# marbl/parsnp

Hardware: AMD Instinct MI355X
Metric: genomes/sec (MUM+LCB end-to-end) (higher is better)
Workload: dtype int32

## Files before the change

parsnp_amd/csrc/engine/engine_core.h:

```cpp
#pragma once
#include <algorithm>
#include <atomic>
#include <chrono>
#include <cstdint>
#include <cstdio>
#include <cstdlib>
#include <cstring>
#include <memory>
#include <mutex>
#include <new>
#include <string>
#include <thread>
#include <vector>

#include "kernels.h"
#include "store_kernels.h"
#include "dense_kernels.h"
#include "index_kernels.h"
#include "snp_kernels.h"

namespace pm {

struct HostPool {
    void* (*alloc_fn)(size_t) = nullptr;
// ... 171 lines not shown
    static constexpr size_t kCtrErr = kCtrBase;
    static constexpr size_t kCtrGrouped = kCtrBase + 2;
    static constexpr size_t kCtrWide = kCtrBase + 3;
    static constexpr size_t kCtrWideWords = 3;
    static constexpr size_t kCtrOverflow = kCtrBase + 6;
    static constexpr size_t kCtrLost = kCtrBase + 7;
    static constexpr size_t kCtrWords = kCtrBase + 8;
    static_assert(kCtrErr < kCtrGrouped && kCtrGrouped < kCtrWide && kCtrWide + kCtrWideWords <= kCtrOverflow && kCtrOverflow < kCtrLost && kCtrLost < kCtrWords,
                  "the words of the counter block are distinct and inside it");

private:
    struct CallHint { int64_t units = 0, ncand = 0, nok = 0; };
    struct StoreCounts { int64_t ms_count, rg_count, layout_rows, rg_pkey_init; };
    StoreCounts store_mark() const { return StoreCounts{ms_count, rg_count, layout_rows, rg_pkey_init}; }
    void store_rewind(const StoreCounts& m) { ms_count = m.ms_count; rg_count = m.rg_count; layout_rows = m.layout_rows; rg_pkey_init = m.rg_pkey_init; }
    void store_reset() { store_rewind(StoreCounts{0, 0, -1, 0}); }

    struct SearchCall {
        const int64_t nreg; const int64_t* const starts; const int64_t* const lens; const int32_t* const minsize; BatchResult* const out;
        const bool want_events, mumi; const GapBatch* const gb;
        bool from_store = false;
        int nq = 0, no_small = 0, lbits = 0;
        size_t nrow = 0, regz = 0, bytes_R = 0, bytes_pre = 0;
        int64_t npairs = 0, npos = 0, tsize = 0, fwords = 0, tsize_clear = 0, fwords_clear = 0, nbk = 0, npos_bucketed = 0, nchunks = 0, centries = 0, nwv = 0;
        RegionInfo* R = nullptr; int64_t *posbase = nullptr, *cbase = nullptr, *stage = nullptr;
        std::vector<int64_t> bbase;
        uint32_t* d_err = nullptr;
        int64_t nflag = 0; uint64_t ovf_cap = 0; bool index_counts_read = false;
        CallHint none; CallHint* hint = nullptr;
        int64_t nunits = 0; bool units_known = false;
        size_t ev_guess = 0, slice_cap = 0, queue_cap = 0, grp_cap = 0;
        uint64_t nev = 0, nrest = 0, ngrp = 0, worst_slice = 0;
        uint32_t errbits = 0, sticky = 0;
        bool first_form = false, wide_form = false, grouping = false, by_buckets = false, sharded = false;
        uint64_t *skey = nullptr, *sval = nullptr;
        const int64_t* ncand_p = nullptr; bool anchor_guess = false;
        bool exact = false, anchor_call = false;
        int64_t ncand_i = 0, nok = 0; uint64_t ncand = 0; size_t nokz = 0; const int64_t* nok_p = nullptr;
        std::vector<uint64_t> counts, qcounts; int64_t nunits_live = 0;
        int32_t verdict = 0;
        std::vector<int32_t> reg_h; int64_t counts_h[2] = {0, 0};
    };
    static constexpr int kNext = 1, kRepeat = 2;

    int run_once(int64_t nreg, const int64_t* starts, const int64_t* lens, const int32_t* minsize, BatchResult* out, bool want_events,
                 bool mumi, const GapBatch* gb = nullptr) {
        SearchCall c{nreg, starts, lens, minsize, out, want_events, mumi, gb};
        int rc = plan_call(c);
        if (rc != kNext) return rc;
        upload_and_clear(c);
        if ((rc = build_index(c)) != kNext) return rc;
        if ((rc = count_units(c)) != kNext) return rc;
        if ((rc = search_events(c)) != kNext) return rc;
        order_events(c);
        if (mumi) return mumi_tail(c);
        if ((rc = master_ep(c)) != kNext) return rc;
        return candidate_tail(c);
    }

    int plan_call(SearchCall& c) {
        const int64_t nreg = c.nreg; const int64_t* const starts = c.starts; const int64_t* const lens = c.lens; const int32_t* const minsize = c.minsize;
        BatchResult* const out = c.out; const GapBatch* const gb = c.gb;
        timing.clear();
        const int nq = c.nq = ngen - 1;
        out->nregions = nreg; out->nq = nq; out->total = 0;
        out->off.assign((size_t)nreg + 1, 0);
        out->release();
// ... 123 lines not shown
    }

    void upload_and_clear(SearchCall& c) {
        const int64_t nreg = c.nreg, npos = c.npos, tsize = c.tsize, fwords = c.fwords, tsize_clear = c.tsize_clear, fwords_clear = c.fwords_clear, npairs = c.npairs, centries = c.centries;
        const int nq = c.nq;
        const size_t nrow = c.nrow, regz = c.regz, bytes_R = c.bytes_R, bytes_pre = c.bytes_pre;
        const GapBatch* const gb = c.gb; const bool from_store = c.from_store;
        RegionInfo* const R = c.R; int64_t* const posbase = c.posbase; int64_t* const cbase = c.cbase; int64_t* const stage = c.stage;
        be.mark("setup");
        ensure(d_R, regz);
        ensure(d_starts, nrow); ensure(d_lens, nrow);
        ensure(d_posbase, regz + 1); ensure(d_cbase, regz + 1);
        be.h2d_staged(d_R.p, R, bytes_R);
        be.h2d_staged(d_posbase.p, posbase, bytes_pre);
        be.h2d_staged(d_cbase.p, cbase, bytes_pre);
        if (!gb) {
            be.h2d_staged(d_starts.p, stage, sizeof(int64_t) * nrow);
            be.h2d_staged(d_lens.p, stage + nrow, sizeof(int64_t) * nrow);
        } else if (from_store) {
            ensure(d_list, regz);
            be.h2d_staged(d_list.p, stage, sizeof(int32_t) * regz);
            be.launch("gather_regions", (int64_t)nrow, GatherRegions{d_list.p, ngen, d_rg_start.p, d_rg_len.p, d_starts.p, d_lens.p});
        }
        ensure(d_counter, kCtrWords);
        uint32_t* d_err = c.d_err = (uint32_t*)(d_counter.p + kCtrErr);

        ensure(d_slots, (size_t)tsize); ensure(d_filter, (size_t)fwords);
        ensure(d_next, (size_t)std::max<int64_t>(npos, 1)); ensure(d_rep, (size_t)std::max<int64_t>(npos, 1));
        ensure(d_epm, (size_t)std::max<int64_t>(npos, 1) + 1);
        const int64_t nwv = c.nwv = (npos + 63) / 64;
        ensure(d_repeated, (size_t)(npos / 32 + 2));
        ensure(d_ucount, (size_t)npairs + 1); ensure(d_uoff, (size_t)npairs + 1);
        ensure(d_coarse, (size_t)std::max<int64_t>(centries, 1));
        ensure(d_wmask, (size_t)nwv + 1); ensure(d_wcount, (size_t)nwv + 1); ensure(d_woff, (size_t)nwv + 1);
        if (from_store) ensure(d_alg, 8 * (size_t)kAlgSets);
        ensure(d_dense, regz);
        {
            const ClearJob jobs[] = {
                {d_filter.p, sizeof(uint32_t) * (size_t)fwords_clear, 0}, {d_slots.p, sizeof(uint64_t) * (size_t)tsize_clear, 0xff}, {d_counter.p, 8 * kCtrWords, 0},
                {d_repeated.p, 4 * (size_t)(npos / 32 + 2), 0}, {d_coarse.p, 4 * (size_t)std::max<int64_t>(centries, 1), 0},
                {d_ucount.p + npairs, 8, 0}, {d_wcount.p + nwv, 8, 0}, {from_store ? d_alg.p : nullptr, from_store ? (size_t)64 * kAlgSets : 0, 0},
                {dense_mode ? nullptr : d_dense.p, dense_mode ? 0 : regz, 0}};
            be.clear_many(jobs, (int)(sizeof jobs / sizeof jobs[0]));
        }
        int64_t& nflag = c.nflag;
        if (dense_mode) {
            for (int64_t r = 0; r < nreg; r++) nflag += dense_h[(size_t)r] ? 1 : 0;
            be.h2d(d_dense.p, dense_h.data(), regz);
            last_dense_regions = nflag;
        }
        if (gb) be.launch("check_rows", (int64_t)nrow, CheckRows{d_R.p, d_starts.p, d_lens.p, ngen, d_glen, d_err});
        if (from_store) {
            be.launch_wave("alg_bytes", (nreg * nq + kAlgPairs - 1) / kAlgPairs, AlgBytes{d_R.p, d_lens.p, ngen, nreg * nq, d_alg.p});
        }
    }

    int build_index(SearchCall& c) {
        const int64_t nreg = c.nreg, npos = c.npos, nbk = c.nbk, npos_bucketed = c.npos_bucketed, nflag = c.nflag;
        const size_t regz = c.regz;
        const RegionInfo* const R = c.R; const std::vector<int64_t>& bbase = c.bbase; uint32_t* const d_err = c.d_err;
        be.mark("index");
        const uint64_t ovf_cap = c.ovf_cap = nbk > 0 ? (uint64_t)(index_overflow_cap > 0 ? index_overflow_cap : npos_bucketed / 32 + 1024) : 0;
        if (nbk > 0) {
            const int pbits = bits_for((uint64_t)npos), bbits = bits_for((uint64_t)nbk);
            if (pbits + bbits > 64) { error = "batch too large for 64-bit index keys"; return -5; }
            ensure(d_bkbase, regz + 1); ensure(d_ikey, (size_t)npos); ensure(d_ikey2, (size_t)npos); ensure(d_bkbegin, (size_t)nbk + 1); ensure(d_ovf, (size_t)ovf_cap);
            be.h2d(d_bkbase.p, bbase.data(), 8 * (regz + 1));
            be.launch("index_keys", npos, IndexKeys{P, d_R.p, nreg, d_posbase.p, d_bkbase.p, pbits, d_ikey.p, d_next.p, d_rep.p});
            if (!sort_keys_on(be, d_ikey.p, d_ikey2.p, (size_t)npos, pbits, pbits + bbits, 0)) {
                ensure(d_ikey3, (size_t)npos); ensure(d_ikey4, (size_t)npos);
                be.launch("index_key_buckets", npos, IndexKeyBuckets{d_ikey.p, pbits, d_ikey3.p});
                be.sort_pairs(d_ikey3.p, d_ikey4.p, d_ikey.p, d_ikey2.p, (size_t)npos, bbits);
            }
// ... 149 lines not shown
        uint32_t& errbits = c.errbits;
        errbits |= c.sticky;
        if (from_store) {
            alg_raw[0] = alg_raw[1] = alg_raw[2] = 0;
            for (int x = 0; x < kAlgSets; x++) for (int k = 0; k < 3; k++) alg_raw[k] += alg_sets[8 * x + k];
        }
        if (from_store) { last_alg[0] = (double)alg_raw[0] / 4.0; last_alg[1] = (double)alg_raw[1] / 2.0; last_alg[2] = (double)alg_raw[2] / 2.0; }
        if (errbits & kErrRows) { error = "region outside its genome"; return -2; }
        rest_cap_hint[nreg == 1] = queue_cap - 64;
        if (gb) hint.units = std::max<int64_t>(nunits_live, 1);
        last_rest = (int64_t)nrest;
        ev_cap_hint = (size_t)(nev + nev / 4);
        if (grouping) grp_cap_hint = (size_t)(ngrp + ngrp / 4);
        last_events = (int64_t)(nev + ngrp);
        last_grouped = (int64_t)ngrp;
        last_grouped_wide = wide_form ? (int64_t)counts[kCtrWide] : 0;
        last_handed_back = wide_form ? (int64_t)counts[kCtrWide + 1] : -1;
        last_wide_regions = wide_form ? (int64_t)counts[kCtrWide + 2] : 0;
        const bool sharded = c.sharded = coll.world > 1 || coll.device;
        if ((errbits & kErrWork) && !sharded) { budget_exceeded = true; error = "per-thread work budget exceeded (degenerate repeat structure in a region)"; return -5; }
        return kNext;
    }

    void order_events(SearchCall& c) {
        const int64_t nreg = c.nreg, npairs = c.npairs, npos = c.npos, nchunks = c.nchunks, centries = c.centries; const int nq = c.nq, lbits = c.lbits;
        const uint64_t ngrp = c.ngrp, worst_slice = c.worst_slice; const size_t slice_cap = c.slice_cap; const bool grouping = c.grouping;
        uint64_t& nev = c.nev;
        ensure(d_evkey2, std::max<size_t>(nev, 1)); ensure(d_evval2, std::max<size_t>(nev, 1));
        ensure_keep(d_evkey3, std::max<size_t>(ngrp + nev, 1), (size_t)ngrp); ensure_keep(d_evval3, std::max<size_t>(ngrp + nev, 1), (size_t)ngrp);
        const int keybits = bits_for((uint64_t)npairs) + lbits + 1;
        uint64_t *skey = c.skey = d_evkey3.p, *sval = c.sval = d_evval3.p;
        const int64_t nbuckets = (int64_t)nq * nchunks;
        const bool by_buckets = c.by_buckets = bucket_sort && nev > 0 && nbuckets < ((int64_t)1 << 31);
        ensure(d_lo, (size_t)npairs + 1);
        if (by_buckets) {
            ensure(d_bcount, (size_t)nbuckets + 1); ensure(d_bbegin, (size_t)nbuckets + 1); ensure(d_pbase, (size_t)npairs);
            int shift = 6;
            while (((uint64_t)1 << shift) < worst_slice) shift++;
            be.memset(d_bcount.p, 0, 8 * ((size_t)nbuckets + 1));
            be.launch("pair_bucket_base", npairs, PairBucketBase{nq, d_cbase.p, d_pbase.p});
            be.launch("event_bucket_count", (int64_t)kSlices << shift, EventBucketCount{d_evkey.p, d_counter.p, (uint64_t)slice_cap, shift, lbits, d_pbase.p, d_bcount.p});
            be.exclusive_scan(d_bcount.p, d_bbegin.p, (size_t)nbuckets + 1);
            be.launch("event_place", (int64_t)kSlices << shift,
                      EventPlace{d_evkey.p, d_evval.p, d_counter.p, (uint64_t)slice_cap, shift, lbits, d_pbase.p, d_bbegin.p, d_bcount.p, d_evkey3.p + ngrp, d_evval3.p + ngrp});
            be.launch("event_order", nbuckets, EventOrder{d_bbegin.p, nbuckets, d_evkey3.p + ngrp, d_evval3.p + ngrp});
        } else if (nev > 0) {
            be.launch("compact_events", (int64_t)nev, CompactEvents{d_evkey.p, d_evval.p, d_sliceoff.p, (uint64_t)slice_cap, d_evkey2.p, d_evval2.p});
            be.sort_pairs(d_evkey2.p, d_evkey3.p + ngrp, d_evval2.p, d_evval3.p + ngrp, (size_t)nev, keybits);
        }
        be.mark("scan");
        const int64_t nev_sorted = (int64_t)nev;
        nev += ngrp;
        if (by_buckets) be.launch("coarse_from_buckets", centries, CoarseFromBuckets{d_bbegin.p, d_cbase.p, nreg, nq, (int64_t)ngrp, d_coarse.p, d_lo.p, npairs, nev_sorted});
        else be.launch("pair_bounds", npairs, PairBounds{skey, (int64_t)nev, lbits, npairs, d_lo.p, (int64_t)ngrp});
        if (grouping) be.launch("grouped_bounds", npairs, GroupedBounds{d_gflag.p, d_glo.p, nq, d_lo.p});
        ensure_keep(d_state, std::max<size_t>(nev, 1), (size_t)ngrp); ensure_keep(d_emax, std::max<size_t>(nev, 1), (size_t)ngrp);
        const int64_t nsorted = (int64_t)(nev - ngrp);
        if (nsorted > 0) {
            const int64_t nwaves = (nsorted + kWaveEvents - 1) / kWaveEvents;
            ensure(d_wsummary, (size_t)nwaves);
            const WaveScanCore core{skey + ngrp, sval + ngrp, nsorted, lbits, d_R.p, nq, d_rep.p};
            be.launch_wave("wave_summary", nwaves, WaveSummary{core, d_wsummary.p});
            be.launch_wave("wave_scan", nwaves, WaveScan{core, d_wsummary.p, d_lo.p, (int64_t)ngrp, d_state.p + ngrp, d_emax.p + ngrp});
        }

        if (c.want_events) {
            ev_key_h.resize((size_t)nev); ev_val_h.resize((size_t)nev); rep_h.resize((size_t)npos);
            if (nev) { be.d2h(ev_key_h.data(), skey, 8 * (size_t)nev); be.d2h(ev_val_h.data(), sval, 8 * (size_t)nev); }
            if (npos) be.d2h(rep_h.data(), d_rep.p, 4 * (size_t)npos);
            ev_lbits = lbits;
        }
    }

    int widest_block() const {
        int widest = 0;
        for (int r = 0; r < coll.world; r++) { int a, b; shard_range(ngen, r, coll.world, &a, &b); widest = std::max(widest, b - a); }
        return std::max(widest, 1);
    }

    int mumi_tail(SearchCall& c) {
        const int64_t npairs = c.npairs; const int lbits = c.lbits; const bool sharded = c.sharded;
        uint64_t* const skey = c.skey; uint64_t* const sval = c.sval; uint32_t& errbits = c.errbits;
        be.mark("mumi_coverage");
        ensure(d_cov, (size_t)npairs);
        be.launch("mumi_coverage", npairs, MumiCoverage{d_R.p, skey, sval, d_lo.p, d_state.p, d_rep.p, lbits, ngen, d_cov.p});
        mumi_covered.resize((size_t)npairs);
        be.d2h(mumi_covered.data(), d_cov.p, 8 * (size_t)npairs);
        if (sharded) {
            const size_t per = (size_t)widest_block() + 1;
            std::vector<int64_t> send(per, 0), recv(per * (size_t)coll.world);
            for (int g = g_first; g < g_last; g++) send[(size_t)(g - g_first)] = mumi_covered[(size_t)(g - 1)];
            send[per - 1] = errbits;
            if (allgather_host(send.data(), (int64_t)(8 * send.size()), recv.data())) { error = "all-gather of MUMi coverage failed"; return -4; }
            for (int r = 0; r < coll.world; r++) {
                int a, b; shard_range(ngen, r, coll.world, &a, &b);
                for (int g = a; g < b; g++) mumi_covered[(size_t)(g - 1)] = recv[(size_t)r * per + (size_t)(g - a)];
// ... 1108 lines not shown
    template <class T> void ensure_keep(Buf<T>& b, size_t n, size_t keep) {
        if (n <= b.cap && b.p) return;
        if (std::find(all_bufs.begin(), all_bufs.end(), (BufBase*)&b) == all_bufs.end()) all_bufs.push_back(&b);
        const size_t want = n + n / 2 + 16;
        void* raw = be.alloc(want * sizeof(T));
        if (!raw) throw DeviceOutOfMemory{want * sizeof(T)};
        if (b.p && keep) { be.d2d(raw, b.p, keep * sizeof(T)); be.sync(); }
        if (b.raw) be.free(b.raw);
        b.raw = raw; b.p = (T*)raw; b.cap = want;
    }
    void collect_timing() { timing = be.collect(); }
    template <class T> static auto group_on(T& b, int) -> decltype(b.d2h_group(), void()) { b.d2h_group(); }
    template <class T> static void group_on(T&, long) {}
    template <class T> static auto flush_on(T& b, int) -> decltype(b.d2h_flush(), void()) { b.d2h_flush(); }
    template <class T> static void flush_on(T&, long) {}
    template <class T> static auto tune_copy_kernel(T& b, bool on, int) -> decltype(b.group_copies = on, true) { b.group_copies = on; return true; }
    template <class T> static bool tune_copy_kernel(T&, bool, long) { return true; }
    template <class T> static auto sort_keys_on(T& b, uint64_t* ki, uint64_t* ko, size_t n, int lo, int hi, int) -> decltype(b.sort_keys(ki, ko, n, lo, hi), true) { b.sort_keys(ki, ko, n, lo, hi); return true; }
    template <class T> static bool sort_keys_on(T&, uint64_t*, uint64_t*, size_t, int, int, long) { return false; }
    void group_downloads() { group_on(be, 0); }
    void flush_downloads() { flush_on(be, 0); }

    SeqBlock* blk = nullptr; int64_t* d_goff = nullptr; int64_t* d_glen = nullptr;
    Packed P{};
    size_t ev_cap_hint = 0, rest_cap_hint[2] = {0, 0}, grp_cap_hint = 0;
    std::vector<CallHint> call_hints;
    int64_t call_ordinal = 0;
    Buf<uint8_t> d_gflag; Buf<int64_t> d_glo;
    Buf<int64_t> d_bkbase, d_bkbegin, d_ovf; Buf<uint64_t> d_ikey, d_ikey2, d_ikey3, d_ikey4;
    Buf<RegionInfo> d_R; Buf<int64_t> d_starts, d_lens, d_posbase;
    Buf<uint64_t> d_slots; Buf<uint32_t> d_filter, d_repeated; Buf<int32_t> d_next, d_rep, d_run, d_epm;
    Buf<int64_t> d_ucount, d_uoff; Buf<UnitRec> d_units;
    Buf<uint64_t> d_counter, d_evkey, d_evval, d_evkey2, d_evval2, d_evkey3, d_evval3; Buf<int64_t> d_sliceoff;
    Buf<int64_t> d_lo, d_cov; Buf<EventAtK> d_state; Buf<PairState> d_wsummary; Buf<int32_t> d_emax;
    Buf<uint64_t> d_cand; Buf<GenomeAtK> d_at; Buf<uint8_t> d_ok; Buf<int32_t> d_ok_k, d_ok_lon, d_osp; Buf<uint8_t> d_ofwd;
    Buf<uint64_t> d_wmask; Buf<int64_t> d_wcount, d_woff;
    Buf<int64_t> d_bcount, d_bbegin, d_pbase;
    Buf<int64_t> d_okcnt, d_okpos, d_cbase; Buf<int32_t> d_coarse; Buf<int32_t> d_creg, d_ck, d_clon, d_csp; Buf<uint8_t> d_cfwd;
    Buf<uint32_t> d_cflags, d_dirty; Buf<int32_t> d_bmax, d_bmin;
    Buf<GenomeAtK> d_xsend, d_xrecv; Buf<uint8_t> d_hsend, d_hrecv;
    Buf<RestItem> d_rest; Buf<uint64_t> d_qcount;
    Buf<uint8_t> d_dense; Buf<int32_t> d_dfi, d_dlist, d_dlcp; Buf<int64_t> d_dstart, d_dhead, d_dfirst;
    Buf<uint64_t> d_dkey, d_dkey2, d_dval, d_dval2; Buf<uint32_t> d_drank[kDenseMaxLevels];
    Buf<int32_t> d_anchor_start, d_anchor_lon; Buf<uint32_t> d_anchor_flags;
    int64_t table_counter = 0;
    Buf<uint64_t> d_image;
    Buf<int64_t> d_un_blk, d_un_cnt, d_un_scan, d_un_tot; Buf<int32_t> d_un_out;
    Buf<uint64_t> d_snp_counts, d_snp_lo, d_snp_hi; Buf<uint8_t> d_snp_chunk; Buf<int64_t> d_snp_flag, d_snp_rank, d_snp_col; Buf<int32_t> d_snp_dist;
    Buf<uint8_t> d_ms_strand, d_ms_state, d_small8, d_o_strand; Buf<int32_t> d_ms_shift, d_ms_len, d_list, d_list2, d_j_min, d_j_max, d_o_start;
    Buf<int64_t> d_rg_start, d_rg_len, d_lay_off, d_lay_bits, d_v_row0, d_v_first, d_f_start, d_f_end, d_f_pack; Buf<RegInfo> d_rg_info; Buf<uint64_t> d_rg_count, d_once, d_twice;
    Buf<RowInfo> d_rowinfo; Buf<uint64_t> d_alg;
    Buf<int64_t> d_sd_cnt, d_sd_off; Buf<uint8_t> d_sd_keep;
    Buf<uint64_t> d_t_rem; Buf<uint8_t> d_t_done;
    Buf<int32_t> d_v_done, d_owner; Buf<uint8_t> d_v_defer, d_v_involved;
    Buf<uint64_t> d_t_left; uint64_t tangle_left[8] = {0, 0, 0, 0, 0, 0, 0, 0}; int tangle_ran = 0;
    Buf<int64_t> d_rg_pkey; Buf<OutsideWrite> d_outw; Buf<uint64_t> d_outw_count; int64_t rg_pkey_init = 0; uint64_t outside_writes_call = 0;
    Buf<ForeignRead> d_foreign; Buf<uint64_t> d_foreign_count, d_foreign_masks; Buf<int64_t> d_ms_key;
    size_t foreign_cap = 0; int64_t ms_key_rows = 0; uint64_t foreign_seen = 0;
    static constexpr size_t kHitCap = 256;
    Buf<uint64_t> d_hit_count, d_hit_owned, d_hit_present; Buf<int32_t> d_hits; Buf<uint8_t> d_recwords;
    Buf<int64_t> d_ch_flag, d_ch_pos, d_ch_head, d_ch_hpos, d_ch_survive, d_ch_spos, d_ch_hdr;
    Buf<uint64_t> d_ch_key, d_ch_val, d_ch_skey, d_ch_srow, d_ch_key2, d_ch_row2, d_ch_lcblen;
    Buf<uint8_t> d_ch_verdict, d_ch_outhead; Buf<int32_t> d_ch_outrow;
    Buf<int64_t> d_ch_back, d_ch_wflag, d_ch_wpos, d_ch_wlist, d_ch_wend; Buf<uint8_t> d_ch_wverdict, d_ch_wkeep;
    uint8_t* chain_host = nullptr; size_t chain_host_cap = 0; void* chain_event = nullptr; bool chain_pending = false; int64_t chain_cap = 0;
    size_t lay_words = 0, rg_cap_hint = 0;
    int64_t layout_rows = -1;
// ... 4 lines not shown
```

parsnp_amd/csrc/engine/kernels.h:

```cpp
#pragma once
#include <cstdint>

#if defined(__HIPCC__)
#define PM_HD __host__ __device__ inline
#else
#define PM_HD inline
#endif

namespace pm {

PM_HD int ctz64(uint64_t x) {
#if defined(__HIP_DEVICE_COMPILE__)
    return __ffsll((unsigned long long)x) - 1;
#else
    return __builtin_ctzll(x);
#endif
}
PM_HD int clz64(uint64_t x) {
#if defined(__HIP_DEVICE_COMPILE__)
    return __clzll((long long)x);
#else
    return __builtin_clzll(x);
#endif
}
// ... 1080 lines not shown

struct PairBucketBase {
    int32_t nq; const int64_t* cbase; int64_t* pbase;
    PM_HD void operator()(int64_t pair) const {
        const int64_t r = pair / nq; const int64_t g = pair % nq;
        pbase[pair] = (int64_t)nq * (cbase[r] - r) + g * (cbase[r + 1] - cbase[r] - 1);
    }
};
PM_HD int64_t bucket_of_key(uint64_t k, int lbits, const int64_t* pbase) {
    return pbase[k >> (lbits + 1)] + (int64_t)(((k >> 1) & ((1ull << lbits) - 1)) >> 8);
}
struct EventBucketCount {
    const uint64_t* key_in; const uint64_t* counters; uint64_t slice_cap; int shift; int lbits; const int64_t* pbase; int64_t* count;
    PM_HD void operator()(int64_t tid) const {
        const uint64_t sl = (uint64_t)tid >> shift, idx = (uint64_t)tid & ((1ull << shift) - 1);
        const bool active = idx < counters[sl * kSliceStride];
#if defined(__HIP_DEVICE_COMPILE__)
        const int lane = (int)__lane_id();
        const int64_t b = active ? bucket_of_key(key_in[sl * slice_cap + idx], lbits, pbase) : -1;
        const int64_t prev = ((int64_t)__shfl_up((int)(b >> 32), 1, 64) << 32) | (uint32_t)__shfl_up((int)(uint32_t)b, 1, 64);
        const bool head = active && (lane == 0 || prev != b);
        const unsigned long long heads = __ballot(head), act = __ballot(active);
        if (!head) return;
        const unsigned long long above = lane == 63 ? 0ull : heads & (~0ull << (lane + 1));
        const int upto = above ? __ffsll((long long)above) - 1 : __popcll(act);
        atomic_add64((uint64_t*)&count[b], (uint64_t)(upto - lane));
#else
        if (active) atomic_add64((uint64_t*)&count[bucket_of_key(key_in[sl * slice_cap + idx], lbits, pbase)], 1);
#endif
    }
};
struct EventPlace {
    const uint64_t* key_in; const uint64_t* val_in; const uint64_t* counters; uint64_t slice_cap; int shift; int lbits; const int64_t* pbase;
    const int64_t* begin; int64_t* count; uint64_t* key_out; uint64_t* val_out;
    PM_HD void operator()(int64_t tid) const {
        const uint64_t sl = (uint64_t)tid >> shift, idx = (uint64_t)tid & ((1ull << shift) - 1);
        const bool active = idx < counters[sl * kSliceStride];
        const uint64_t src = sl * slice_cap + idx;
#if defined(__HIP_DEVICE_COMPILE__)
        const int lane = (int)__lane_id();
        const uint64_t k = active ? key_in[src] : 0;
        const int64_t b = active ? bucket_of_key(k, lbits, pbase) : -1;
        const int64_t prev = ((int64_t)__shfl_up((int)(b >> 32), 1, 64) << 32) | (uint32_t)__shfl_up((int)(uint32_t)b, 1, 64);
        const bool head = active && (lane == 0 || prev != b);
        const unsigned long long heads = __ballot(head), act = __ballot(active);
        int64_t first = 0;
        if (head) {
            const unsigned long long above = lane == 63 ? 0ull : heads & (~0ull << (lane + 1));
            const int upto = above ? __ffsll((long long)above) - 1 : __popcll(act);
            const int64_t run = upto - lane;
            first = begin[b] + (int64_t)atomic_add64((uint64_t*)&count[b], (uint64_t)(-run)) - run;
        }
        const unsigned long long below = heads & (lane == 63 ? ~0ull : ((2ull << lane) - 1));
        const int mine = below ? 63 - __clzll((long long)below) : 0;
        first = ((int64_t)__shfl((int)(first >> 32), mine, 64) << 32) | (uint32_t)__shfl((int)(uint32_t)first, mine, 64);
        if (!active) return;
        const int64_t at = first + (lane - mine);
        key_out[at] = k; val_out[at] = val_in[src];
#else
        if (!active) return;
        const uint64_t k = key_in[src];
        const int64_t b = bucket_of_key(k, lbits, pbase);
        const int64_t at = begin[b] + (int64_t)atomic_add64((uint64_t*)&count[b], ~0ull) - 1;
        key_out[at] = k; val_out[at] = val_in[src];
#endif
    }
};
struct EventOrder {
    const int64_t* begin; int64_t nbuckets; uint64_t* key; uint64_t* val;
    PM_HD void operator()(int64_t b) const {
        const int64_t a = begin[b], n = begin[b + 1] - a;
        if (n < 2) return;
        uint64_t* k = key + a; uint64_t* v = val + a;
        if (n == 2) {
            const uint64_t k0 = k[0], k1 = k[1];
            if (k1 < k0) { const uint64_t v0 = v[0], v1 = v[1]; k[0] = k1; k[1] = k0; v[0] = v1; v[1] = v0; }
            return;
        }
        if (n <= 8) {
            uint64_t rk[8], rv[8];
#pragma unroll
            for (int i = 0; i < 8; i++) { rk[i] = i < n ? k[i] : ~0ull; rv[i] = i < n ? v[i] : 0; }
#define PM_CX(a, b) { const bool sw = rk[b] < rk[a]; const uint64_t ka = sw ? rk[b] : rk[a], kb = sw ? rk[a] : rk[b], va = sw ? rv[b] : rv[a], vb = sw ? rv[a] : rv[b]; rk[a] = ka; rk[b] = kb; rv[a] = va; rv[b] = vb; }
            PM_CX(0, 1) PM_CX(2, 3) PM_CX(4, 5) PM_CX(6, 7)
            PM_CX(0, 2) PM_CX(1, 3) PM_CX(4, 6) PM_CX(5, 7)
            PM_CX(1, 2) PM_CX(5, 6) PM_CX(0, 4) PM_CX(3, 7)
            PM_CX(1, 5) PM_CX(2, 6)
            PM_CX(1, 4) PM_CX(3, 6)
            PM_CX(2, 4) PM_CX(3, 5)
            PM_CX(3, 4)
#undef PM_CX
#pragma unroll
            for (int i = 0; i < 8; i++) if (i < n) { k[i] = rk[i]; v[i] = rv[i]; }
            return;
        }
        int64_t gap = 1;
        while (gap < n / 3) gap = 3 * gap + 1;
        for (; gap >= 1; gap /= 3)
            for (int64_t i = gap; i < n; i++) {
                const uint64_t kk = k[i], vv = v[i];
                int64_t j = i;
                while (j >= gap && k[j - gap] > kk) { k[j] = k[j - gap]; v[j] = v[j - gap]; j -= gap; }
                k[j] = kk; v[j] = vv;
            }
    }
};
struct CoarseFromBuckets {
    const int64_t* begin; const int64_t* cbase; int64_t nregions; int32_t nq; int64_t base; int32_t* coarse; int64_t* lo; int64_t npairs; int64_t total;
    PM_HD void operator()(int64_t tid) const {
        const int64_t row = tid / nq; const int64_t g = tid % nq;
        int64_t a = 0, z = nregions;
        while (z - a > 1) { const int64_t mid = (a + z) >> 1; if (cbase[mid] <= row) a = mid; else z = mid; }
        const int64_t r = a, b = row - cbase[r], blocks = cbase[r + 1] - cbase[r] - 1;
        const int64_t first = (int64_t)nq * (cbase[r] - r) + g * blocks;
        const int64_t f = begin[first];
        coarse[tid] = (int32_t)(begin[first + b] - f);
        if (b == 0) lo[r * nq + g] = base + f;
        if (tid == 0) lo[npairs] = base + total;
    }
};

struct PairBounds {
    const uint64_t* key; int64_t nev; int lbits; int64_t npairs; int64_t* lo;
    int64_t base;
    PM_HD void operator()(int64_t pair) const {
        uint64_t want = (uint64_t)pair << (lbits + 1);
        int64_t a = base, b = nev;
        while (a < b) { int64_t mid = (a + b) >> 1; if (key[mid] < want) a = mid + 1; else b = mid; }
        lo[pair] = a;
        if (pair == npairs - 1) lo[npairs] = nev;
    }
};
struct StrandAtK { int32_t e1, up, spb; };
struct EventAtK { StrandAtK s[2]; };
#ifndef PM_WAVE_EVENTS
#define PM_WAVE_EVENTS 512
#endif
constexpr int kWaveEvents = PM_WAVE_EVENTS;
struct WinState { int32_t e1, e2, wl, wj, wr; };
struct PairState { WinState s[2]; };
PM_HD WinState win_join(const WinState& a, const WinState& b) {
    if (a.e1 == 0) return b;
    if (b.e1 == 0) return a;
    const bool a_wins = a.e1 > b.e1 || (a.e1 == b.e1 && (a.wl < b.wl || (a.wl == b.wl && a.wj <= b.wj)));
    WinState o;
    if (a_wins) { o = a; o.e2 = a.e2 > b.e1 ? a.e2 : b.e1; }
    else { o = b; o.e2 = b.e2 > a.e1 ? b.e2 : a.e1; }
    return o;
}
PM_HD PairState pair_join(const PairState& a, const PairState& b) { PairState o; o.s[0] = win_join(a.s[0], b.s[0]); o.s[1] = win_join(a.s[1], b.s[1]); return o; }
PM_HD PairState pair_of_event(uint64_t k, uint64_t v, uint64_t lmask, int32_t rp) {
    const int32_t l = (int32_t)((k >> 1) & lmask), j = (int32_t)(v >> 32);
    PairState o; o.s[0] = WinState{0, 0, 0, 0, 0}; o.s[1] = o.s[0];
    const WinState w{l + (int32_t)(v & 0xffffffffu), 0, l, j, rp};
    if (k & 1) o.s[1] = w; else o.s[0] = w;
    return o;
}
PM_HD EventAtK resolved(const PairState& p) {
    EventAtK o;
    for (int sd = 0; sd < 2; sd++) {
        const WinState& w = p.s[sd];
        const int32_t up = w.wl + w.wr;
        o.s[sd] = w.e1 ? StrandAtK{w.e1, w.e2 > up ? w.e2 : up, w.wj - w.wl} : StrandAtK{0, 0, 0};
    }
    return o;
}
#if defined(__HIP_DEVICE_COMPILE__)
__device__ inline WinState win_shfl_up(const WinState& x, int d) { return WinState{__shfl_up(x.e1, d, 64), __shfl_up(x.e2, d, 64), __shfl_up(x.wl, d, 64), __shfl_up(x.wj, d, 64), __shfl_up(x.wr, d, 64)}; }
__device__ inline WinState win_bcast(const WinState& x, int lane) { return WinState{__shfl(x.e1, lane, 64), __shfl(x.e2, lane, 64), __shfl(x.wl, lane, 64), __shfl(x.wj, lane, 64), __shfl(x.wr, lane, 64)}; }
__device__ inline bool pair_scan(PairState& x, bool head) {
    const int lane = (int)__lane_id();
    int h = head ? 1 : 0;
    for (int d = 1; d < 64; d <<= 1) {
        PairState y; y.s[0] = win_shfl_up(x.s[0], d); y.s[1] = win_shfl_up(x.s[1], d);
        const int hy = __shfl_up(h, d, 64);
        if (lane >= d && !h) { x = pair_join(y, x); h = hy; }
    }
    return h != 0;
}
#endif
struct WaveScanCore {
    const uint64_t* key; const uint64_t* val; int64_t nev; int lbits; const RegionInfo* R; int32_t nq; const int32_t* rep;
    PM_HD PairState run(int64_t w, PairState carry, bool store, EventAtK* st, int32_t* emax, bool* opened) const {
        const uint64_t lmask = (1ull << lbits) - 1;
        const int64_t a = w * kWaveEvents, b = a + kWaveEvents < nev ? a + kWaveEvents : nev;
        bool any_head = false;
#if defined(__HIP_DEVICE_COMPILE__)
        const int lane = (int)__lane_id();
        for (int64_t base = a; base < b; base += 64) {
            const int64_t i = base + lane;
            const bool in = i < b;
            PairState x; x.s[0] = WinState{0, 0, 0, 0, 0}; x.s[1] = x.s[0];
            bool head = false;
            if (in) {
                const uint64_t k = key[i], v = val[i];
                const uint64_t pair = k >> (lbits + 1);
                head = i == 0 || (key[i - 1] >> (lbits + 1)) != pair;
                x = pair_of_event(k, v, lmask, store ? rep[R[(int64_t)pair / nq].posbase + (int32_t)((k >> 1) & lmask)] : 0);
            }
            const bool h = pair_scan(x, head);
            if (!h) x = pair_join(carry, x);
            if (in && store) { st[i] = resolved(x); emax[i] = x.s[0].e1 > x.s[1].e1 ? x.s[0].e1 : x.s[1].e1; }
            const int last = (int)((b - base < 64 ? b - base : 64) - 1);
            carry.s[0] = win_bcast(x.s[0], last); carry.s[1] = win_bcast(x.s[1], last);
            any_head = any_head || __ballot(head) != 0;
        }
#else
        for (int64_t i = a; i < b; i++) {
            const uint64_t k = key[i], v = val[i];
            const uint64_t pair = k >> (lbits + 1);
            const bool head = i == 0 || (key[i - 1] >> (lbits + 1)) != pair;
            const PairState x = pair_of_event(k, v, lmask, store ? rep[R[(int64_t)pair / nq].posbase + (int32_t)((k >> 1) & lmask)] : 0);
            carry = head ? x : pair_join(carry, x);
            any_head = any_head || head;
            if (store) { st[i] = resolved(carry); emax[i] = carry.s[0].e1 > carry.s[1].e1 ? carry.s[0].e1 : carry.s[1].e1; }
        }
#endif
        if (opened) *opened = any_head;
        return carry;
    }
};
struct WaveSummary {
    WaveScanCore core; PairState* summary;
    PM_HD void wave(int64_t w) const {
        PairState none; none.s[0] = WinState{0, 0, 0, 0, 0}; none.s[1] = none.s[0];
        PairState t = core.run(w, none, false, nullptr, nullptr, nullptr);
        if (wave_leader_k()) {
            const int64_t b = (w + 1) * kWaveEvents < core.nev ? (w + 1) * kWaveEvents : core.nev;
            const int64_t posbase = core.R[(int64_t)(core.key[b - 1] >> (core.lbits + 1)) / core.nq].posbase;
            if (t.s[0].e1) t.s[0].wr = core.rep[posbase + t.s[0].wl];
            if (t.s[1].e1) t.s[1].wr = core.rep[posbase + t.s[1].wl];
            summary[w] = t;
        }
    }
};
struct WaveScan {
    WaveScanCore core; const PairState* summary; const int64_t* lo; int64_t lo_base; EventAtK* st; int32_t* emax;
    PM_HD void wave(int64_t w) const {
        PairState carry; carry.s[0] = WinState{0, 0, 0, 0, 0}; carry.s[1] = carry.s[0];
        const int64_t a = w * kWaveEvents;
        const uint64_t pair = core.key[a] >> (core.lbits + 1);
        if (a > 0 && (core.key[a - 1] >> (core.lbits + 1)) == pair) {
            const int64_t s0 = (lo[pair] - lo_base) / kWaveEvents;
            for (int64_t p = s0; p < w; p++) carry = pair_join(carry, summary[p]);
        }
        (void)core.run(w, carry, true, st, emax, nullptr);
    }
};

struct MumiCoverage {
    const RegionInfo* R; const uint64_t* key; const uint64_t* val; const int64_t* lo; const EventAtK* st; const int32_t* rep;
    int lbits; int32_t ngen; int64_t* covered;
    PM_HD void operator()(int64_t pair) const {
        const RegionInfo& ri = R[pair / (ngen - 1)];
        const uint64_t lmask = (1ull << lbits) - 1;
        int32_t last_ep = 0, cov_end = 0; int64_t cov = 0;
        const int64_t a = lo[pair], b = lo[pair + 1];
        for (int64_t i = a; i < b; i++) {
            int32_t l = (int32_t)((key[i] >> 1) & lmask);
            int32_t lnext = i + 1 < b ? (int32_t)((key[i + 1] >> 1) & lmask) : ri.nR;
            if (lnext == l) continue;
            const EventAtK& s = st[i];
            const int32_t ep[2] = {s.s[0].e1, s.s[1].e1}, up[2] = {s.s[0].up, s.s[1].up};
            int c = ep[0] > ep[1] ? 0 : 1;
            int32_t EP = ep[c], UP = up[c];
            if (!(EP > last_ep && UP < EP)) continue;
            int32_t k = l;
            if (!(EP - k < ri.nR)) { k = l + 1; if (k >= lnext || k >= ri.nR) continue; }
            last_ep = EP;
            if (EP - k >= 15) {
                int32_t from = k > cov_end ? k : cov_end;
                if (EP > from) cov += EP - from;
                if (EP > cov_end) cov_end = EP;
            }
        }
        covered[pair] = cov;
    }
};

// ... 431 lines not shown
```

Measured before the change: 31010.

## Parallelize wave-scan carry, tile coarse_from_buckets, and simplify bucket placement cursors

Several changes to the event-ordering pipeline. The wave summary now reduces only the last pair's events with a wave-wide shuffle reduction, and a new SummaryCarry kernel computes per-wave carries in tiles. This replaces the serial per-wave loop over prior summaries that was quadratic for long pairs. CoarseFromBuckets becomes a wave-tiled kernel staging through shared memory for coalesced writes, EventPlace uses a single forward cursor array offset by one instead of begin+count decrement, the coarse clear is deferred or skipped when buckets rebuild it, and win_join is made branchless. Together these add an extra kernel launch and more complex indexing logic in exchange.

```diff
diff --git a/parsnp_amd/csrc/engine/engine_core.h b/parsnp_amd/csrc/engine/engine_core.h
--- a/parsnp_amd/csrc/engine/engine_core.h
+++ b/parsnp_amd/csrc/engine/engine_core.h
@@ -227,7 +227,7 @@
         size_t ev_guess = 0, slice_cap = 0, queue_cap = 0, grp_cap = 0;
         uint64_t nev = 0, nrest = 0, ngrp = 0, worst_slice = 0;
         uint32_t errbits = 0, sticky = 0;
-        bool first_form = false, wide_form = false, grouping = false, by_buckets = false, sharded = false;
+        bool first_form = false, wide_form = false, grouping = false, by_buckets = false, coarse_by_buckets = false, sharded = false;
         uint64_t *skey = nullptr, *sval = nullptr;
         const int64_t* ncand_p = nullptr; bool anchor_guess = false;
         bool exact = false, anchor_call = false;
@@ -417,13 +417,14 @@
         ensure(d_repeated, (size_t)(npos / 32 + 2));
         ensure(d_ucount, (size_t)npairs + 1); ensure(d_uoff, (size_t)npairs + 1);
         ensure(d_coarse, (size_t)std::max<int64_t>(centries, 1));
+        c.coarse_by_buckets = bucket_sort && (int64_t)c.nq * c.nchunks < ((int64_t)1 << 31);
         ensure(d_wmask, (size_t)nwv + 1); ensure(d_wcount, (size_t)nwv + 1); ensure(d_woff, (size_t)nwv + 1);
         if (from_store) ensure(d_alg, 8 * (size_t)kAlgSets);
         ensure(d_dense, regz);
         {
             const ClearJob jobs[] = {
                 {d_filter.p, sizeof(uint32_t) * (size_t)fwords_clear, 0}, {d_slots.p, sizeof(uint64_t) * (size_t)tsize_clear, 0xff}, {d_counter.p, 8 * kCtrWords, 0},
-                {d_repeated.p, 4 * (size_t)(npos / 32 + 2), 0}, {d_coarse.p, 4 * (size_t)std::max<int64_t>(centries, 1), 0},
+                {d_repeated.p, 4 * (size_t)(npos / 32 + 2), 0}, {c.coarse_by_buckets ? nullptr : d_coarse.p, c.coarse_by_buckets ? 0 : 4 * (size_t)std::max<int64_t>(centries, 1), 0},
                 {d_ucount.p + npairs, 8, 0}, {d_wcount.p + nwv, 8, 0}, {from_store ? d_alg.p : nullptr, from_store ? (size_t)64 * kAlgSets : 0, 0},
                 {dense_mode ? nullptr : d_dense.p, dense_mode ? 0 : regz, 0}};
             be.clear_many(jobs, (int)(sizeof jobs / sizeof jobs[0]));
@@ -639,17 +640,18 @@
         uint64_t *skey = c.skey = d_evkey3.p, *sval = c.sval = d_evval3.p;
         const int64_t nbuckets = (int64_t)nq * nchunks;
         const bool by_buckets = c.by_buckets = bucket_sort && nev > 0 && nbuckets < ((int64_t)1 << 31);
+        if (c.coarse_by_buckets && !by_buckets) be.memset(d_coarse.p, 0, 4 * (size_t)std::max<int64_t>(centries, 1));
         ensure(d_lo, (size_t)npairs + 1);
         if (by_buckets) {
-            ensure(d_bcount, (size_t)nbuckets + 1); ensure(d_bbegin, (size_t)nbuckets + 1); ensure(d_pbase, (size_t)npairs);
+            ensure(d_bcount, (size_t)nbuckets + 2); ensure(d_bbegin, (size_t)nbuckets + 2); ensure(d_pbase, (size_t)npairs);
             int shift = 6;
             while (((uint64_t)1 << shift) < worst_slice) shift++;
-            be.memset(d_bcount.p, 0, 8 * ((size_t)nbuckets + 1));
+            be.memset(d_bcount.p, 0, 8 * ((size_t)nbuckets + 2));
             be.launch("pair_bucket_base", npairs, PairBucketBase{nq, d_cbase.p, d_pbase.p});
-            be.launch("event_bucket_count", (int64_t)kSlices << shift, EventBucketCount{d_evkey.p, d_counter.p, (uint64_t)slice_cap, shift, lbits, d_pbase.p, d_bcount.p});
-            be.exclusive_scan(d_bcount.p, d_bbegin.p, (size_t)nbuckets + 1);
+            be.launch("event_bucket_count", (int64_t)kSlices << shift, EventBucketCount{d_evkey.p, d_counter.p, (uint64_t)slice_cap, shift, lbits, d_pbase.p, d_bcount.p + 1});
+            be.exclusive_scan(d_bcount.p, d_bbegin.p, (size_t)nbuckets + 2);
             be.launch("event_place", (int64_t)kSlices << shift,
-                      EventPlace{d_evkey.p, d_evval.p, d_counter.p, (uint64_t)slice_cap, shift, lbits, d_pbase.p, d_bbegin.p, d_bcount.p, d_evkey3.p + ngrp, d_evval3.p + ngrp});
+                      EventPlace{d_evkey.p, d_evval.p, d_counter.p, (uint64_t)slice_cap, shift, lbits, d_pbase.p, d_bbegin.p + 1, d_evkey3.p + ngrp, d_evval3.p + ngrp});
             be.launch("event_order", nbuckets, EventOrder{d_bbegin.p, nbuckets, d_evkey3.p + ngrp, d_evval3.p + ngrp});
         } else if (nev > 0) {
             be.launch("compact_events", (int64_t)nev, CompactEvents{d_evkey.p, d_evval.p, d_sliceoff.p, (uint64_t)slice_cap, d_evkey2.p, d_evval2.p});
@@ -658,17 +660,18 @@
         be.mark("scan");
         const int64_t nev_sorted = (int64_t)nev;
         nev += ngrp;
-        if (by_buckets) be.launch("coarse_from_buckets", centries, CoarseFromBuckets{d_bbegin.p, d_cbase.p, nreg, nq, (int64_t)ngrp, d_coarse.p, d_lo.p, npairs, nev_sorted});
+        if (by_buckets) be.launch_wave("coarse_from_buckets", coarse_tiles(centries / nq, nq), CoarseFromBuckets{d_bbegin.p, d_cbase.p, nreg, nq, (int64_t)ngrp, d_coarse.p, d_lo.p, npairs, nev_sorted, centries / nq});
         else be.launch("pair_bounds", npairs, PairBounds{skey, (int64_t)nev, lbits, npairs, d_lo.p, (int64_t)ngrp});
         if (grouping) be.launch("grouped_bounds", npairs, GroupedBounds{d_gflag.p, d_glo.p, nq, d_lo.p});
         ensure_keep(d_state, std::max<size_t>(nev, 1), (size_t)ngrp); ensure_keep(d_emax, std::max<size_t>(nev, 1), (size_t)ngrp);
         const int64_t nsorted = (int64_t)(nev - ngrp);
         if (nsorted > 0) {
             const int64_t nwaves = (nsorted + kWaveEvents - 1) / kWaveEvents;
-            ensure(d_wsummary, (size_t)nwaves);
+            ensure(d_wsummary, (size_t)nwaves); ensure(d_wcarry, (size_t)nwaves);
             const WaveScanCore core{skey + ngrp, sval + ngrp, nsorted, lbits, d_R.p, nq, d_rep.p};
             be.launch_wave("wave_summary", nwaves, WaveSummary{core, d_wsummary.p});
-            be.launch_wave("wave_scan", nwaves, WaveScan{core, d_wsummary.p, d_lo.p, (int64_t)ngrp, d_state.p + ngrp, d_emax.p + ngrp});
+            be.launch_wave("summary_carry", (nwaves + kCarryTiles - 1) / kCarryTiles, SummaryCarry{core, d_wsummary.p, nwaves, d_lo.p, (int64_t)ngrp, d_wcarry.p});
+            be.launch_wave("wave_scan", nwaves, WaveScan{core, d_wcarry.p, d_state.p + ngrp, d_emax.p + ngrp});
         }
 
         if (c.want_events) {
@@ -1843,7 +1846,7 @@
     Buf<uint64_t> d_slots; Buf<uint32_t> d_filter, d_repeated; Buf<int32_t> d_next, d_rep, d_run, d_epm;
     Buf<int64_t> d_ucount, d_uoff; Buf<UnitRec> d_units;
     Buf<uint64_t> d_counter, d_evkey, d_evval, d_evkey2, d_evval2, d_evkey3, d_evval3; Buf<int64_t> d_sliceoff;
-    Buf<int64_t> d_lo, d_cov; Buf<EventAtK> d_state; Buf<PairState> d_wsummary; Buf<int32_t> d_emax;
+    Buf<int64_t> d_lo, d_cov; Buf<EventAtK> d_state; Buf<PairState> d_wsummary, d_wcarry; Buf<int32_t> d_emax;
     Buf<uint64_t> d_cand; Buf<GenomeAtK> d_at; Buf<uint8_t> d_ok; Buf<int32_t> d_ok_k, d_ok_lon, d_osp; Buf<uint8_t> d_ofwd;
     Buf<uint64_t> d_wmask; Buf<int64_t> d_wcount, d_woff;
     Buf<int64_t> d_bcount, d_bbegin, d_pbase;
diff --git a/parsnp_amd/csrc/engine/kernels.h b/parsnp_amd/csrc/engine/kernels.h
--- a/parsnp_amd/csrc/engine/kernels.h
+++ b/parsnp_amd/csrc/engine/kernels.h
@@ -1136,7 +1136,7 @@
 };
 struct EventPlace {
     const uint64_t* key_in; const uint64_t* val_in; const uint64_t* counters; uint64_t slice_cap; int shift; int lbits; const int64_t* pbase;
-    const int64_t* begin; int64_t* count; uint64_t* key_out; uint64_t* val_out;
+    int64_t* cursor; uint64_t* key_out; uint64_t* val_out;
     PM_HD void operator()(int64_t tid) const {
         const uint64_t sl = (uint64_t)tid >> shift, idx = (uint64_t)tid & ((1ull << shift) - 1);
         const bool active = idx < counters[sl * kSliceStride];
@@ -1152,8 +1152,7 @@
         if (head) {
             const unsigned long long above = lane == 63 ? 0ull : heads & (~0ull << (lane + 1));
             const int upto = above ? __ffsll((long long)above) - 1 : __popcll(act);
-            const int64_t run = upto - lane;
-            first = begin[b] + (int64_t)atomic_add64((uint64_t*)&count[b], (uint64_t)(-run)) - run;
+            first = (int64_t)atomic_add64((uint64_t*)&cursor[b], (uint64_t)(upto - lane));
         }
         const unsigned long long below = heads & (lane == 63 ? ~0ull : ((2ull << lane) - 1));
         const int mine = below ? 63 - __clzll((long long)below) : 0;
@@ -1164,8 +1163,7 @@
 #else
         if (!active) return;
         const uint64_t k = key_in[src];
-        const int64_t b = bucket_of_key(k, lbits, pbase);
-        const int64_t at = begin[b] + (int64_t)atomic_add64((uint64_t*)&count[b], ~0ull) - 1;
+        const int64_t at = (int64_t)atomic_add64((uint64_t*)&cursor[bucket_of_key(k, lbits, pbase)], 1);
         key_out[at] = k; val_out[at] = val_in[src];
 #endif
     }
@@ -1209,18 +1207,76 @@
             }
     }
 };
+constexpr int kCoarseRows = 32, kCoarseGen = 64;
+PM_HD int64_t coarse_tiles(int64_t nrows, int32_t nq) { return ((nrows + kCoarseRows - 1) / kCoarseRows) * ((nq + kCoarseGen - 1) / kCoarseGen); }
 struct CoarseFromBuckets {
-    const int64_t* begin; const int64_t* cbase; int64_t nregions; int32_t nq; int64_t base; int32_t* coarse; int64_t* lo; int64_t npairs; int64_t total;
-    PM_HD void operator()(int64_t tid) const {
-        const int64_t row = tid / nq; const int64_t g = tid % nq;
+    const int64_t* begin; const int64_t* cbase; int64_t nregions; int32_t nq; int64_t base; int32_t* coarse; int64_t* lo; int64_t npairs; int64_t total; int64_t nrows;
+    PM_HD int64_t region_of_row(int64_t row) const {
         int64_t a = 0, z = nregions;
         while (z - a > 1) { const int64_t mid = (a + z) >> 1; if (cbase[mid] <= row) a = mid; else z = mid; }
-        const int64_t r = a, b = row - cbase[r], blocks = cbase[r + 1] - cbase[r] - 1;
-        const int64_t first = (int64_t)nq * (cbase[r] - r) + g * blocks;
-        const int64_t f = begin[first];
-        coarse[tid] = (int32_t)(begin[first + b] - f);
-        if (b == 0) lo[r * nq + g] = base + f;
-        if (tid == 0) lo[npairs] = base + total;
+        return a;
+    }
+    PM_HD void wave(int64_t w) const {
+        const int64_t gtiles = (nq + kCoarseGen - 1) / kCoarseGen;
+        const int64_t row0 = (w / gtiles) * kCoarseRows; const int32_t g0 = (int32_t)(w % gtiles) * kCoarseGen;
+        const int rows = (int)(nrows - row0 < kCoarseRows ? nrows - row0 : kCoarseRows), gens = nq - g0 < kCoarseGen ? nq - g0 : kCoarseGen;
+#if defined(__HIP_DEVICE_COMPILE__)
+        __shared__ int32_t s_v[kCoarseGen][kCoarseRows + 1];
+        __shared__ int64_t s_f[kCoarseGen];
+        __shared__ int64_t s_reg[kCoarseRows], s_cb[kCoarseRows], s_blocks[kCoarseRows];
+        const int lane = (int)__lane_id();
+        if (w == 0 && lane == 0) lo[npairs] = base + total;
+        if (lane < rows) {
+            const int64_t r = region_of_row(row0 + lane);
+            s_reg[lane] = r; s_cb[lane] = cbase[r]; s_blocks[lane] = cbase[r + 1] - cbase[r] - 1;
+        }
+        __syncthreads();
+        if (s_reg[0] == s_reg[rows - 1]) {
+            const int64_t r = s_reg[0], cb = s_cb[0], blocks = s_blocks[0], b0 = row0 - cb;
+            const int64_t pairs0 = (int64_t)nq * (cb - r);
+            if (lane < gens) {
+                const int64_t f = begin[pairs0 + (int64_t)(g0 + lane) * blocks];
+                s_f[lane] = f;
+                if (b0 == 0) lo[r * nq + g0 + lane] = base + f;
+            }
+            __syncthreads();
+            const int bl = lane & (kCoarseRows - 1);
+            for (int gl = lane / kCoarseRows; gl < gens; gl += 64 / kCoarseRows)
+                if (bl < rows) s_v[gl][bl] = (int32_t)(begin[pairs0 + (int64_t)(g0 + gl) * blocks + b0 + bl] - s_f[gl]);
+            __syncthreads();
+            if (lane < gens)
+                for (int x = 0; x < rows; x++) coarse[(row0 + x) * nq + g0 + lane] = s_v[lane][x];
+        } else if (lane < gens) {
+            constexpr int kAtOnce = 8;
+            for (int x0 = 0; x0 < rows; x0 += kAtOnce) {
+                int64_t f[kAtOnce]; int32_t v[kAtOnce];
+#pragma unroll
+                for (int t = 0; t < kAtOnce; t++) {
+                    const int x = x0 + t < rows ? x0 + t : rows - 1;
+                    const int64_t first = (int64_t)nq * (s_cb[x] - s_reg[x]) + (int64_t)(g0 + lane) * s_blocks[x];
+                    f[t] = begin[first]; v[t] = (int32_t)(begin[first + (row0 + x - s_cb[x])] - f[t]);
+                }
+#pragma unroll
+                for (int t = 0; t < kAtOnce; t++)
+                    if (x0 + t < rows) {
+                        const int x = x0 + t;
+                        coarse[(row0 + x) * nq + g0 + lane] = v[t];
+                        if (row0 + x == s_cb[x]) lo[s_reg[x] * nq + g0 + lane] = base + f[t];
+                    }
+            }
+        }
+#else
+        if (w == 0) lo[npairs] = base + total;
+        for (int x = 0; x < rows; x++) {
+            const int64_t row = row0 + x, r = region_of_row(row), b = row - cbase[r], blocks = cbase[r + 1] - cbase[r] - 1;
+            for (int32_t g = g0; g < g0 + gens; g++) {
+                const int64_t first = (int64_t)nq * (cbase[r] - r) + (int64_t)g * blocks;
+                const int64_t f = begin[first];
+                coarse[row * nq + g] = (int32_t)(begin[first + b] - f);
+                if (b == 0) lo[r * nq + g] = base + f;
+            }
+        }
+#endif
     }
 };
 
@@ -1244,13 +1300,9 @@
 struct WinState { int32_t e1, e2, wl, wj, wr; };
 struct PairState { WinState s[2]; };
 PM_HD WinState win_join(const WinState& a, const WinState& b) {
-    if (a.e1 == 0) return b;
-    if (b.e1 == 0) return a;
-    const bool a_wins = a.e1 > b.e1 || (a.e1 == b.e1 && (a.wl < b.wl || (a.wl == b.wl && a.wj <= b.wj)));
-    WinState o;
-    if (a_wins) { o = a; o.e2 = a.e2 > b.e1 ? a.e2 : b.e1; }
-    else { o = b; o.e2 = b.e2 > a.e1 ? b.e2 : a.e1; }
-    return o;
+    const bool a_wins = b.e1 == 0 || (a.e1 != 0 && (a.e1 > b.e1 || (a.e1 == b.e1 && (a.wl < b.wl || (a.wl == b.wl && a.wj <= b.wj)))));
+    const int32_t second = a_wins ? a.e2 : b.e2, loser = a_wins ? b.e1 : a.e1;
+    return WinState{a_wins ? a.e1 : b.e1, second > loser ? second : loser, a_wins ? a.wl : b.wl, a_wins ? a.wj : b.wj, a_wins ? a.wr : b.wr};
 }
 PM_HD PairState pair_join(const PairState& a, const PairState& b) { PairState o; o.s[0] = win_join(a.s[0], b.s[0]); o.s[1] = win_join(a.s[1], b.s[1]); return o; }
 PM_HD PairState pair_of_event(uint64_t k, uint64_t v, uint64_t lmask, int32_t rp) {
@@ -1282,73 +1334,128 @@
     }
     return h != 0;
 }
-#endif
+__device__ inline PairState pair_reduce(PairState x) {
+    for (int d = 32; d >= 1; d >>= 1) {
+        PairState y;
+        for (int sd = 0; sd < 2; sd++)
+            y.s[sd] = WinState{__shfl_xor(x.s[sd].e1, d, 64), __shfl_xor(x.s[sd].e2, d, 64), __shfl_xor(x.s[sd].wl, d, 64), __shfl_xor(x.s[sd].wj, d, 64), __shfl_xor(x.s[sd].wr, d, 64)};
+        x = pair_join(x, y);
+    }
+    return x;
+}
+#endif
+PM_HD PairState pair_none() { PairState o; o.s[0] = WinState{0, 0, 0, 0, 0}; o.s[1] = o.s[0]; return o; }
+PM_HD int64_t region_of_pair(uint64_t pair, int32_t nq) { return (int64_t)((uint32_t)pair / (uint32_t)nq); }
+constexpr int kCarryTiles = 16;
 struct WaveScanCore {
     const uint64_t* key; const uint64_t* val; int64_t nev; int lbits; const RegionInfo* R; int32_t nq; const int32_t* rep;
-    PM_HD PairState run(int64_t w, PairState carry, bool store, EventAtK* st, int32_t* emax, bool* opened) const {
+    PM_HD uint64_t pair_at(int64_t i) const { return key[i] >> (lbits + 1); }
+    PM_HD int64_t end_of(int64_t w) const { return (w + 1) * kWaveEvents < nev ? (w + 1) * kWaveEvents : nev; }
+    PM_HD PairState sequential(int64_t w, PairState carry, bool store, EventAtK* st, int32_t* emax) const {
         const uint64_t lmask = (1ull << lbits) - 1;
-        const int64_t a = w * kWaveEvents, b = a + kWaveEvents < nev ? a + kWaveEvents : nev;
-        bool any_head = false;
-#if defined(__HIP_DEVICE_COMPILE__)
+        const int64_t a = w * kWaveEvents, b = end_of(w);
+        for (int64_t i = a; i < b; i++) {
+            const uint64_t k = key[i], v = val[i];
+            const uint64_t pair = k >> (lbits + 1);
+            const bool head = i == 0 || pair_at(i - 1) != pair;
+            const PairState x = pair_of_event(k, v, lmask, store ? rep[R[region_of_pair(pair, nq)].posbase + (int32_t)((k >> 1) & lmask)] : 0);
+            carry = head ? x : pair_join(carry, x);
+            if (store) { st[i] = resolved(carry); emax[i] = carry.s[0].e1 > carry.s[1].e1 ? carry.s[0].e1 : carry.s[1].e1; }
+        }
+        return carry;
+    }
+};
+struct WaveSummary {
+    WaveScanCore core; PairState* summary;
+    PM_HD void wave(int64_t w) const {
+        const int64_t a = w * kWaveEvents, b = core.end_of(w);
+        const uint64_t last = core.pair_at(b - 1);
+#if defined(__HIP_DEVICE_COMPILE__)
+        const uint64_t lmask = (1ull << core.lbits) - 1;
         const int lane = (int)__lane_id();
+        PairState t = pair_none();
+        constexpr int rounds = (kWaveEvents + 63) / 64;
+        uint64_t k[rounds], v[rounds];
+#pragma unroll
+        for (int x = 0; x < rounds; x++) {
+            const int64_t i = a + 64 * x + lane;
+            const int64_t at = i < b ? i : b - 1;
+            k[x] = core.key[at]; v[x] = core.val[at];
+        }
+#pragma unroll
+        for (int x = 0; x < rounds; x++)
+            if (a + 64 * x + lane < b && (k[x] >> (core.lbits + 1)) == last) t = pair_join(t, pair_of_event(k[x], v[x], lmask, 0));
+        t = pair_reduce(t);
+#else
+        PairState t = core.sequential(w, pair_none(), false, nullptr, nullptr);
+#endif
+        if (wave_leader_k()) {
+            const int64_t posbase = core.R[region_of_pair(last, core.nq)].posbase;
+            if (t.s[0].e1) t.s[0].wr = core.rep[posbase + t.s[0].wl];
+            if (t.s[1].e1) t.s[1].wr = core.rep[posbase + t.s[1].wl];
+            summary[w] = t;
+        }
+    }
+};
+struct SummaryCarry {
+    WaveScanCore core; const PairState* summary; int64_t nwaves; const int64_t* lo; int64_t lo_base; PairState* carry;
+    PM_HD bool continues(int64_t w) const { return w > 0 && core.pair_at(w * kWaveEvents - 1) == core.pair_at(w * kWaveEvents); }
+    PM_HD bool opens(int64_t w) const { return w == 0 || core.pair_at(w * kWaveEvents - 1) != core.pair_at(core.end_of(w) - 1); }
+    PM_HD void wave(int64_t c) const {
+        const int64_t w0 = c * kCarryTiles;
+        const int64_t s0 = continues(w0) ? (lo[core.pair_at(w0 * kWaveEvents)] - lo_base) / kWaveEvents : w0;
+#if defined(__HIP_DEVICE_COMPILE__)
+        const int lane = (int)__lane_id();
+        PairState into = pair_none();
+        for (int64_t p = s0 + lane; p < w0; p += 64) into = pair_join(into, summary[p]);
+        if (s0 < w0) into = pair_reduce(into);
+        const int64_t w = w0 + lane;
+        const bool in = lane < kCarryTiles && w < nwaves;
+        PairState x = in ? summary[w] : pair_none();
+        const bool h = pair_scan(x, in && opens(w));
+        if (!h) x = pair_join(into, x);
+        PairState before;
+        before.s[0] = win_shfl_up(x.s[0], 1); before.s[1] = win_shfl_up(x.s[1], 1);
+        if (lane == 0) before = into;
+        if (in) carry[w] = continues(w) ? before : pair_none();
+#else
+        PairState run = pair_none();
+        for (int64_t p = s0; p < w0; p++) run = pair_join(run, summary[p]);
+        for (int64_t w = w0; w < w0 + kCarryTiles && w < nwaves; w++) {
+            carry[w] = continues(w) ? run : pair_none();
+            run = opens(w) ? summary[w] : pair_join(run, summary[w]);
+        }
+#endif
+    }
+};
+struct WaveScan {
+    WaveScanCore core; const PairState* carry; EventAtK* st; int32_t* emax;
+    PM_HD void wave(int64_t w) const {
+#if defined(__HIP_DEVICE_COMPILE__)
+        const uint64_t lmask = (1ull << core.lbits) - 1;
+        const int lane = (int)__lane_id();
+        const int64_t a = w * kWaveEvents, b = core.end_of(w);
+        PairState into = carry[w];
         for (int64_t base = a; base < b; base += 64) {
             const int64_t i = base + lane;
             const bool in = i < b;
-            PairState x; x.s[0] = WinState{0, 0, 0, 0, 0}; x.s[1] = x.s[0];
+            PairState x = pair_none();
             bool head = false;
             if (in) {
-                const uint64_t k = key[i], v = val[i];
-                const uint64_t pair = k >> (lbits + 1);
-                head = i == 0 || (key[i - 1] >> (lbits + 1)) != pair;
-                x = pair_of_event(k, v, lmask, store ? rep[R[(int64_t)pair / nq].posbase + (int32_t)((k >> 1) & lmask)] : 0);
+                const uint64_t k = core.key[i], v = core.val[i];
+                const uint64_t pair = k >> (core.lbits + 1);
+                head = i == 0 || core.pair_at(i - 1) != pair;
+                x = pair_of_event(k, v, lmask, core.rep[core.R[region_of_pair(pair, core.nq)].posbase + (int32_t)((k >> 1) & lmask)]);
             }
             const bool h = pair_scan(x, head);
-            if (!h) x = pair_join(carry, x);
-            if (in && store) { st[i] = resolved(x); emax[i] = x.s[0].e1 > x.s[1].e1 ? x.s[0].e1 : x.s[1].e1; }
+            if (!h) x = pair_join(into, x);
+            if (in) { st[i] = resolved(x); emax[i] = x.s[0].e1 > x.s[1].e1 ? x.s[0].e1 : x.s[1].e1; }
             const int last = (int)((b - base < 64 ? b - base : 64) - 1);
-            carry.s[0] = win_bcast(x.s[0], last); carry.s[1] = win_bcast(x.s[1], last);
-            any_head = any_head || __ballot(head) != 0;
-        }
-#else
-        for (int64_t i = a; i < b; i++) {
-            const uint64_t k = key[i], v = val[i];
-            const uint64_t pair = k >> (lbits + 1);
-            const bool head = i == 0 || (key[i - 1] >> (lbits + 1)) != pair;
-            const PairState x = pair_of_event(k, v, lmask, store ? rep[R[(int64_t)pair / nq].posbase + (int32_t)((k >> 1) & lmask)] : 0);
-            carry = head ? x : pair_join(carry, x);
-            any_head = any_head || head;
-            if (store) { st[i] = resolved(carry); emax[i] = carry.s[0].e1 > carry.s[1].e1 ? carry.s[0].e1 : carry.s[1].e1; }
-        }
-#endif
-        if (opened) *opened = any_head;
-        return carry;
-    }
-};
-struct WaveSummary {
-    WaveScanCore core; PairState* summary;
-    PM_HD void wave(int64_t w) const {
-        PairState none; none.s[0] = WinState{0, 0, 0, 0, 0}; none.s[1] = none.s[0];
-        PairState t = core.run(w, none, false, nullptr, nullptr, nullptr);
-        if (wave_leader_k()) {
-            const int64_t b = (w + 1) * kWaveEvents < core.nev ? (w + 1) * kWaveEvents : core.nev;
-            const int64_t posbase = core.R[(int64_t)(core.key[b - 1] >> (core.lbits + 1)) / core.nq].posbase;
-            if (t.s[0].e1) t.s[0].wr = core.rep[posbase + t.s[0].wl];
-            if (t.s[1].e1) t.s[1].wr = core.rep[posbase + t.s[1].wl];
-            summary[w] = t;
-        }
-    }
-};
-struct WaveScan {
-    WaveScanCore core; const PairState* summary; const int64_t* lo; int64_t lo_base; EventAtK* st; int32_t* emax;
-    PM_HD void wave(int64_t w) const {
-        PairState carry; carry.s[0] = WinState{0, 0, 0, 0, 0}; carry.s[1] = carry.s[0];
-        const int64_t a = w * kWaveEvents;
-        const uint64_t pair = core.key[a] >> (core.lbits + 1);
-        if (a > 0 && (core.key[a - 1] >> (core.lbits + 1)) == pair) {
-            const int64_t s0 = (lo[pair] - lo_base) / kWaveEvents;
-            for (int64_t p = s0; p < w; p++) carry = pair_join(carry, summary[p]);
-        }
-        (void)core.run(w, carry, true, st, emax, nullptr);
+            into.s[0] = win_bcast(x.s[0], last); into.s[1] = win_bcast(x.s[1], last);
+        }
+#else
+        (void)core.sequential(w, carry[w], true, st, emax);
+#endif
     }
 };
 
```

After: 31810 (median of 6 runs). 1.03x the previous value.
